# yccyenchicheng/p2pvg

Hardware: NVIDIA H100
Metric: frames/sec (train step, device-timed) MovingMNIST 64x64 seq30 (higher is better)
Workload: dtype bf16

## Files before the change

### p2pvg_b200/csrc/conv_gemm.cu

```cuda
#include <cstdlib>
#include <mutex>

#include "tc_common.cuh"

namespace {

using namespace tc;

constexpr int BLOCK_M = 128;
constexpr int NUM_THREADS = 384;
constexpr int A_STAGE_BYTES = BLOCK_M * 128;

template <int BN> struct Cfg {
  static constexpr int B_STAGE_BYTES = BN * 128;
  static constexpr int STAGE_BYTES = A_STAGE_BYTES + B_STAGE_BYTES;
  static constexpr int STAGES = (BN == 128) ? 4 : 7;
  static constexpr int ACC_LD = BN + 4;
  static constexpr int ACC_BYTES = BLOCK_M * ACC_LD * 4;
  static constexpr int SMEM_BYTES = STAGES * STAGE_BYTES + ACC_BYTES + 1024 + 512;
};

struct Geom {
  int N, H, W;
  int Ck, Cn;
  int M;
  int Ntot;
  int bh128, bn128;
  int bh64, bn64;
  int bw64;
  int imgs_per_group;
  int add_bf16;
  int bres;
  int swap;
  int ks, st, sgn;
};

__device__ __forceinline__ void pix_block(int pb, int P, int H, int W, int bh, int bn, int& n0, int& y0) {
  const int HW = H * W;
  if (HW >= P) {
    const int bpi = HW / P;
    n0 = pb / bpi;
    y0 = (pb - n0 * bpi) * bh;
  } else {
    n0 = pb * bn;
    y0 = 0;
  }
}

__device__ __forceinline__ void addend_load64(float4 (&a4)[16], const float* base, long long elem_off, bool is_bf16) {
  if (is_bf16) {
    const uint4* p = reinterpret_cast<const uint4*>(reinterpret_cast<const bf16*>(base) + elem_off);
#pragma unroll
    for (int j = 0; j < 8; j++) {
      const uint4 r = p[j];
      a4[j] = make_float4(__uint_as_float(r.x), __uint_as_float(r.y), __uint_as_float(r.z), __uint_as_float(r.w));
    }
  } else {
    const float4* p = reinterpret_cast<const float4*>(base + elem_off);
#pragma unroll
    for (int j = 0; j < 16; j++) a4[j] = p[j];
  }
}
__device__ __forceinline__ void addend_add32(float (&f)[32], const float4 (&a4)[16], int h, bool is_bf16) {
  if (is_bf16) {
#pragma unroll
    for (int j = 0; j < 4; j++) {
      const float4 r = a4[4 * h + j];
      float v[8];
      unpack16<bf16>(make_uint4(__float_as_uint(r.x), __float_as_uint(r.y), __float_as_uint(r.z), __float_as_uint(r.w)), v);
#pragma unroll
      for (int i = 0; i < 8; i++) f[8 * j + i] += v[i];
    }
  } else {
#pragma unroll
    for (int j = 0; j < 8; j++) {
      const float4 x4 = a4[8 * h + j];
      f[4 * j] += x4.x; f[4 * j + 1] += x4.y; f[4 * j + 2] += x4.z; f[4 * j + 3] += x4.w;
    }
  }
}

template <int KIND, int BN, bool STAT, bool EVAL = false>
__global__ void __launch_bounds__(NUM_THREADS, 1)
conv_gemm_kernel(const __grid_constant__ CUtensorMap tmA, const __grid_constant__ CUtensorMap tmB, void* __restrict__ Cv, int c_bf16,
                 long long ldc, Geom g, int accumulate, const float* __restrict__ bias, const float* __restrict__ addend,
                 const int* __restrict__ grp_src, float* __restrict__ partial, int kb_per_split, int splits,
                 float2* __restrict__ stat_partial, const float* __restrict__ eval_scale, const float* __restrict__ eval_shift, int act) {
  using C_ = Cfg<BN>;
  constexpr bool A_MN = (KIND == 1), B_MN = (KIND != 0);
  extern __shared__ uint8_t smem_raw[];
  uint8_t* smem = reinterpret_cast<uint8_t*>((reinterpret_cast<uintptr_t>(smem_raw) + 1023) & ~(uintptr_t)1023);
  float* accs = reinterpret_cast<float*>(smem + C_::STAGES * C_::STAGE_BYTES);
  uint64_t* full_bar = reinterpret_cast<uint64_t*>(smem + C_::STAGES * C_::STAGE_BYTES + C_::ACC_BYTES);
  uint64_t* empty_bar = full_bar + C_::STAGES;
  uint64_t* acc_full_bar = empty_bar + C_::STAGES;
  uint64_t* acc_empty_bar = acc_full_bar + 1;
  uint64_t* bres_bar = acc_empty_bar + 1;
  const bool bres = (KIND == 0) && (BN == 64) && g.bres != 0;
  constexpr int BRES_B_BYTES = 9 * 64 * 128, BRES_STAGES = 6;
  static_assert(BN != 64 || BRES_B_BYTES + BRES_STAGES * A_STAGE_BYTES <= C_::STAGES * C_::STAGE_BYTES, "resident weights + A ring");

  const int warp = threadIdx.x >> 5, lane = threadIdx.x & 31;
  const int tiles_m = (g.M + BLOCK_M - 1) / BLOCK_M, tiles_n = (g.Ntot + BN - 1) / BN;
  const int tiles_mn = tiles_m * tiles_n;
  const int phases = (KIND == 2) ? 4 : 1;
  const int num_tiles = tiles_mn * splits * phases;
  const int cchunks = g.Ck / 64;
  const int nkb_total = (KIND == 0) ? g.ks * g.ks * cchunks : (KIND == 2) ? 4 * cchunks : (g.N * g.H * g.W + 63) / 64;

  if (threadIdx.x == 0) {
    for (int s = 0; s < C_::STAGES; s++) {
      mbar_init(&full_bar[s], 1);
      mbar_init(&empty_bar[s], 128);
    }
    mbar_init(acc_full_bar, 128);
    mbar_init(acc_empty_bar, 4);
    mbar_init(bres_bar, 1);
    asm volatile("fence.mbarrier_init.release.cluster;" ::: "memory");
  }
  __syncthreads();

  if (warp >= 8) {
    regs_producer();
    if (warp == 8 && lane == 0) {
      uint32_t it = 0;
      if (bres) {
        mbar_expect_tx(bres_bar, (uint32_t)(g.ks * g.ks) * 64 * 128);
        for (int tap = 0; tap < g.ks * g.ks; tap++) tma_load_2d(&tmB, bres_bar, smem + tap * 64 * 128, tap * 64, 0);
      }
      for (int t = blockIdx.x; t < num_tiles; t += gridDim.x) {
        const int ph = (KIND == 2) ? (t & 3) : 0;
        const int t2 = (KIND == 2) ? (t >> 2) : t;
        const int z = (splits == 1) ? 0 : t2 / tiles_mn, r = t2 - z * tiles_mn;
        const int mt = (tiles_n == 1) ? r : r / tiles_n, nt = (tiles_n == 1) ? 0 : r - mt * tiles_n;
        const int n0 = nt * BN;
        const int kb0 = z * kb_per_split, kb1 = min(kb0 + kb_per_split, nkb_total);
        int pn0 = 0, py0 = 0;
        if (KIND != 1) pix_block(mt, 128, g.H, g.W, g.bh128, g.bn128, pn0, py0);
        const int pa = ph >> 1, pb_ = ph & 1;
        int kn0 = 0, ky0 = 0, kx0 = 0;
        int t_kh = 0, t_kw = 0, t_cc = 0;
        int qc0[BN / 64], qdx[BN / 64], qdy[BN / 64];
        int mc0[2] = {0, 0}, mdx[2] = {0, 0}, mdy[2] = {0, 0};
        if (KIND == 1) {
          if (g.bw64 < g.W) {
            const int per_row = g.W / g.bw64;
            const int rowi = kb0 / per_row;
            kx0 = (kb0 - rowi * per_row) * g.bw64;
            kn0 = rowi / g.H;
            ky0 = rowi - kn0 * g.H;
          } else {
            pix_block(kb0, 64, g.H, g.W, g.bh64, g.bn64, kn0, ky0);
          }
#pragma unroll
          for (int q = 0; q < BN / 64; q++) {
            const int nb = n0 + 64 * q;
            const int tap = nb / g.Cn;
            const int kh = tap / g.ks;
            qc0[q] = nb - tap * g.Cn;
            qdx[q] = tap - kh * g.ks - 1;
            qdy[q] = kh - 1;
          }
          if (g.swap) {
#pragma unroll
            for (int q = 0; q < 2; q++) {
              const int mb = mt * BLOCK_M + 64 * q;
              int tap = mb / g.Cn;
              if (tap >= g.ks * g.ks) tap = g.ks * g.ks - 1;
              const int kh = tap / g.ks;
              mc0[q] = mb < g.M ? mb - tap * g.Cn : 0;
              mdx[q] = tap - kh * g.ks - 1;
              mdy[q] = kh - 1;
            }
          }
        }
        for (int kb = kb0; kb < kb1; kb++, it++) {
          const int s = bres ? (int)(it % BRES_STAGES) : (int)(it % C_::STAGES);
          const uint32_t par = (bres ? (it / BRES_STAGES) : (it / C_::STAGES)) & 1;
          mbar_wait(&empty_bar[s], par ^ 1);
          uint8_t* sa = bres ? smem + BRES_B_BYTES + s * A_STAGE_BYTES : smem + s * C_::STAGE_BYTES;
          uint8_t* sb = sa + A_STAGE_BYTES;
          mbar_expect_tx(&full_bar[s], bres ? A_STAGE_BYTES : C_::STAGE_BYTES);
          if (KIND == 0) {
            tma_load_4d(&tmA, &full_bar[s], sa, t_cc * 64, g.sgn * (t_kw - 1), g.st * py0 + g.sgn * (t_kh - 1), pn0);
            if (!bres) tma_load_2d(&tmB, &full_bar[s], sb, kb * 64, n0);
            if (++t_cc == cchunks) { t_cc = 0; if (++t_kw == g.ks) { t_kw = 0; t_kh++; } }
          } else if (KIND == 2) {
            const int tq = t_kh, c0 = t_cc * 64;
            if (++t_cc == cchunks) { t_cc = 0; t_kh++; }
            const int i = tq >> 1, j = tq & 1;
            const int dy = i == 0 ? 0 : (pa ? 1 : -1), ky = i == 0 ? pa + 1 : (pa ? 0 : 3);
            const int dx = j == 0 ? 0 : (pb_ ? 1 : -1), kx = j == 0 ? pb_ + 1 : (pb_ ? 0 : 3);
            tma_load_4d(&tmA, &full_bar[s], sa, c0, dx, py0 + dy, pn0);
#pragma unroll
            for (int q = 0; q < BN / 64; q++)
              tma_load_2d(&tmB, &full_bar[s], sb + q * 64 * 128, (ky * 4 + kx) * g.Cn + n0 + 64 * q, c0);
          } else {
            const int m0 = mt * BLOCK_M;
            if (g.swap) {
              tma_load_4d(&tmA, &full_bar[s], sa, mc0[0], g.st * kx0 + mdx[0], g.st * ky0 + mdy[0], kn0);
              tma_load_4d(&tmA, &full_bar[s], sa + 64 * 128, mc0[1], g.st * kx0 + mdx[1], g.st * ky0 + mdy[1], kn0);
#pragma unroll
              for (int q = 0; q < BN / 64; q++) tma_load_2d(&tmB, &full_bar[s], sb + q * 64 * 128, n0 + 64 * q, kb * 64);
            } else {
              tma_load_2d(&tmA, &full_bar[s], sa, m0, kb * 64);
              tma_load_2d(&tmA, &full_bar[s], sa + 64 * 128, m0 + 64, kb * 64);
#pragma unroll
              for (int q = 0; q < BN / 64; q++)
                tma_load_4d(&tmB, &full_bar[s], sb + q * 64 * 128, qc0[q], g.st * kx0 + qdx[q], g.st * ky0 + qdy[q], kn0);
            }
            if (g.bw64 < g.W) {
              kx0 += g.bw64;
              if (kx0 >= g.W) { kx0 = 0; if (++ky0 >= g.H) { ky0 = 0; kn0++; } }
            } else if (g.H * g.W >= 64) {
              ky0 += g.bh64;
              if (ky0 >= g.H) { ky0 = 0; kn0++; }
            } else {
              kn0 += g.bn64;
            }
          }
        }
      }
    }
  } else if (warp >= 4) {
    regs_worker();
    const int wt = threadIdx.x - 128;
    const uint32_t smem0 = smem_u32(smem);
    const uint64_t da0 = A_MN ? make_desc(smem0, 64 * 128, 1024) : make_desc(smem0, 0, 1024);
    const uint64_t db0 = B_MN ? make_desc(smem0 + A_STAGE_BYTES, 64 * 128, 1024) : make_desc(smem0 + A_STAGE_BYTES, 0, 1024);
    uint32_t it = 0, lt = 0;
    if (bres) mbar_wait(bres_bar, 0);
    const uint64_t da0r = make_desc(smem0 + BRES_B_BYTES, 0, 1024), db0r = make_desc(smem0, 0, 1024);
    float acc[2][BN / 2];
    for (int t = blockIdx.x; t < num_tiles; t += gridDim.x, lt++) {
      int z = 0;
      if (splits > 1) z = t / tiles_mn;
      const int kb0 = z * kb_per_split, kb1 = min(kb0 + kb_per_split, nkb_total);
      int prev = -1;
      for (int kb = kb0; kb < kb1; kb++, it++) {
        const int s = bres ? (int)(it % BRES_STAGES) : (int)(it % C_::STAGES);
        const uint32_t par = (bres ? (it / BRES_STAGES) : (it / C_::STAGES)) & 1;
        mbar_wait(&full_bar[s], par);
        const uint64_t stage_off = (uint64_t)((uint32_t)s * (uint32_t)(C_::STAGE_BYTES >> 4));
        const uint64_t a_off = bres ? (uint64_t)((uint32_t)s * (uint32_t)(A_STAGE_BYTES >> 4)) : stage_off;
        const uint64_t b_off = bres ? (uint64_t)((uint32_t)kb * (uint32_t)((64 * 128) >> 4)) : stage_off;
        fence_regs(acc[0]);
        fence_regs(acc[1]);
        wgmma_fence();
        wgmma_kblock<false, BN, A_MN, B_MN>(acc, (bres ? da0r : da0) + a_off, (bres ? db0r : db0) + b_off, kb == kb0);
        wgmma_commit();
        wgmma_wait<1>();
        fence_regs(acc[0]);
        fence_regs(acc[1]);
        if (prev >= 0) mbar_arrive(&empty_bar[prev]);
        prev = s;
      }
      wgmma_wait<0>();
      fence_regs(acc[0]);
      fence_regs(acc[1]);
      if (prev >= 0) mbar_arrive(&empty_bar[prev]);
      mbar_wait(acc_empty_bar, (lt & 1) ^ 1);
      acc_to_smem<BN>(acc, accs, C_::ACC_LD, wt);
      mbar_arrive(acc_full_bar);
    }
  } else {
    regs_worker();
    const int q = warp;
    __shared__ float bias_s[2 * BN];
    __shared__ float2 stat_s[STAT ? 2 * 4 * BN : 1];
    constexpr bool do_stat = STAT;
    __shared__ float ev_s[EVAL ? 2 * 2 * BN : 1];
    uint32_t lt = 0;
    for (int t = blockIdx.x; t < num_tiles; t += gridDim.x, lt++) {
      const int ph = (KIND == 2) ? (t & 3) : 0;
      const int t2 = (KIND == 2) ? (t >> 2) : t;
      const int z = (splits == 1) ? 0 : t2 / tiles_mn, r = t2 - z * tiles_mn;
      const int mt = (tiles_n == 1) ? r : r / tiles_n, nt = (tiles_n == 1) ? 0 : r - mt * tiles_n;
      const int n0 = nt * BN;
      const uint32_t acc = lt & 1;
      const int rt = q * 32 + lane;
      long long out_row = (long long)mt * BLOCK_M + rt;
      long long add_row = 0;
      bool row_ok = out_row < g.M;
      if (KIND == 2) {
        int pn0, py0;
        pix_block(mt, 128, g.H, g.W, g.bh128, g.bn128, pn0, py0);
        const int HW = g.H * g.W;
        int nn, yy, xx;
        if (HW >= 128) { nn = 0; yy = rt / g.W; xx = rt - yy * g.W; }
        else { nn = rt / HW; const int rem = rt - nn * HW; yy = rem / g.W; xx = rem - yy * g.W; }
        const int n = pn0 + nn, y = py0 + yy;
        row_ok = (n < g.N) && (y < g.H);
        const int oy = 2 * y + (ph >> 1), ox = 2 * xx + (ph & 1);
        out_row = ((long long)n * (2 * g.H) + oy) * (2 * g.W) + ox;
        if (addend && row_ok) {
          const int n2 = grp_src[n / g.imgs_per_group] * g.imgs_per_group + (n % g.imgs_per_group);
          add_row = ((long long)n2 * (2 * g.H) + oy) * (2 * g.W) + ox;
        }
      }
      if (KIND == 0 && addend && row_ok) {
        const int HW = g.H * g.W;
        const int n = (int)(out_row / HW);
        const int n2 = grp_src[n / g.imgs_per_group] * g.imgs_per_group + (n % g.imgs_per_group);
        add_row = (long long)n2 * HW + (out_row - (long long)n * HW);
      }
      if (EVAL) {
        for (int i = q * 32 + lane; i < BN; i += 128) {
          const bool in = n0 + i < g.Ntot;
          ev_s[acc * 2 * BN + i] = in ? eval_scale[n0 + i] : 0.f;
          ev_s[acc * 2 * BN + BN + i] = in ? eval_shift[n0 + i] : 0.f;
        }
        if (bias == nullptr) epi_bar_sync();
      }
      if (bias != nullptr) {
        for (int i = q * 32 + lane; i < BN; i += 128) bias_s[acc * BN + i] = (n0 + i < g.Ntot) ? bias[n0 + i] : 0.f;
        epi_bar_sync();
      }
      const bool use_add = (KIND != 1) && addend != nullptr && row_ok;
      const long long aoff0 = add_row * g.Ntot + n0;
      const bool abf = g.add_bf16 != 0;
      float4 a4[16];
      if (use_add) addend_load64(a4, addend, aoff0, abf);
      mbar_wait(acc_full_bar, lt & 1);
#pragma unroll 1
      for (int pr = 0; pr < BN / 64; pr++) {
        if (pr > 0 && use_add) addend_load64(a4, addend, aoff0 + pr * 64, abf);
#pragma unroll
        for (int h = 0; h < 2; h++) {
          const int c = pr * 2 + h;
          uint32_t v[32];
          acc_row32(accs + rt * C_::ACC_LD + c * 32, v);
          if (c == BN / 32 - 1) {
            __syncwarp();
            if (lane == 0) mbar_arrive(acc_empty_bar);
          }
          const int nbase = n0 + c * 32;
          if (nbase >= g.Ntot) continue;
          if (!row_ok && !do_stat) continue;
          if (KIND == 1 && partial != nullptr) {
            float* dst = partial + ((long long)z * g.M + out_row) * g.Ntot + nbase;
#pragma unroll
            for (int j = 0; j < 32; j += 8)
              st_global_256(dst + j, v[j], v[j + 1], v[j + 2], v[j + 3], v[j + 4], v[j + 5], v[j + 6], v[j + 7]);
            continue;
          }
          float f[32];
#pragma unroll
          for (int j = 0; j < 32; j++) f[j] = __uint_as_float(v[j]);
          if (bias) {
            const float* bs = bias_s + acc * BN + c * 32;
#pragma unroll
            for (int j = 0; j < 32; j += 4) {
              const float4 b4 = *reinterpret_cast<const float4*>(bs + j);
              f[j] += b4.x; f[j + 1] += b4.y; f[j + 2] += b4.z; f[j + 3] += b4.w;
            }
          }
          if (use_add) addend_add32(f, a4, h, abf);
          if (EVAL) {
            const float* sc = ev_s + acc * 2 * BN + c * 32;
#pragma unroll
            for (int j = 0; j < 32; j++) {
              float y = fmaf(f[j], sc[j], sc[BN + j]);
              if (act == P2PVG_ACT_LRELU) y = y > 0.f ? y : 0.2f * y;
              else if (act == P2PVG_ACT_TANH) y = tanhf(y);
              f[j] = y;
            }
          }
          if (STAT) {
            float s1[32], s2[32];
#pragma unroll
            for (int j = 0; j < 32; j++) {
              const float r = row_ok ? (c_bf16 ? bf16_round(f[j]) : f[j]) : 0.f;
              s1[j] = r;
              s2[j] = r * r;
            }
            const float cs = warp_colsum32(s1, lane), cq = warp_colsum32(s2, lane);
            stat_s[(acc * 4 + q) * BN + c * 32 + lane] = make_float2(cs, cq);
            if (!row_ok) continue;
          }
          if (c_bf16) {
            bf16* crow = reinterpret_cast<bf16*>(Cv) + out_row * ldc + nbase;
            if (accumulate) {
#pragma unroll
              for (int j = 0; j < 32; j++) f[j] += __bfloat162float(crow[j]);
            }
            if ((reinterpret_cast<uintptr_t>(crow) & 31) == 0) {
#pragma unroll
              for (int j = 0; j < 32; j += 16)
                st_global_256(crow + j, pack_bf16x2(f[j], f[j + 1]), pack_bf16x2(f[j + 2], f[j + 3]), pack_bf16x2(f[j + 4], f[j + 5]),
                              pack_bf16x2(f[j + 6], f[j + 7]), pack_bf16x2(f[j + 8], f[j + 9]), pack_bf16x2(f[j + 10], f[j + 11]),
                              pack_bf16x2(f[j + 12], f[j + 13]), pack_bf16x2(f[j + 14], f[j + 15]));
            } else {
#pragma unroll
              for (int j = 0; j < 32; j += 8) {
                uint4 pk;
                pk.x = pack_bf16x2(f[j], f[j + 1]);
                pk.y = pack_bf16x2(f[j + 2], f[j + 3]);
                pk.z = pack_bf16x2(f[j + 4], f[j + 5]);
                pk.w = pack_bf16x2(f[j + 6], f[j + 7]);
                *reinterpret_cast<uint4*>(crow + j) = pk;
              }
            }
          } else {
            float* crow = reinterpret_cast<float*>(Cv) + out_row * ldc + nbase;
            if (accumulate) {
#pragma unroll
              for (int j = 0; j < 32; j++) f[j] += crow[j];
            }
            if ((reinterpret_cast<uintptr_t>(crow) & 31) == 0) {
#pragma unroll
              for (int j = 0; j < 32; j += 8)
                st_global_256(crow + j, __float_as_uint(f[j]), __float_as_uint(f[j + 1]), __float_as_uint(f[j + 2]), __float_as_uint(f[j + 3]),
                              __float_as_uint(f[j + 4]), __float_as_uint(f[j + 5]), __float_as_uint(f[j + 6]), __float_as_uint(f[j + 7]));
            } else {
#pragma unroll
              for (int j = 0; j < 32; j += 4) *reinterpret_cast<float4*>(crow + j) = make_float4(f[j], f[j + 1], f[j + 2], f[j + 3]);
            }
          }
        }
      }
      if (STAT) {
        epi_bar_sync();
        float2* dst = stat_partial + ((long long)mt * phases + ph) * g.Ntot + n0;
        for (int i = q * 32 + lane; i < BN; i += 128) {
          if (n0 + i >= g.Ntot) continue;
          const float2 a = stat_s[(acc * 4 + 0) * BN + i], b = stat_s[(acc * 4 + 1) * BN + i];
          const float2 c2 = stat_s[(acc * 4 + 2) * BN + i], d = stat_s[(acc * 4 + 3) * BN + i];
          dst[i] = make_float2((a.x + b.x) + (c2.x + d.x), (a.y + b.y) + (c2.y + d.y));
        }
      }
    }
  }
}

__global__ void conv_splitk_reduce_kernel(const float* __restrict__ partial, int splits, float* __restrict__ C, long long ldc, int M, int N,
                                          int accumulate, int transposed) {
  const long long total = (long long)M * N;
  for (long long idx = (long long)blockIdx.x * blockDim.x + threadIdx.x; idx < total; idx += (long long)gridDim.x * blockDim.x) {
    const long long m = idx / N;
    const int n = (int)(idx - m * N);
    const long long pidx = transposed ? (long long)n * M + m : idx;
    float acc = 0.f;
    for (int z = 0; z < splits; z++) acc += partial[(long long)z * total + pidx];
    if (accumulate) acc += C[m * ldc + n];
    C[m * ldc + n] = acc;
  }
}

typedef CUresult (*EncodeTiledFn)(CUtensorMap*, CUtensorMapDataType, cuuint32_t, void*, const cuuint64_t*, const cuuint64_t*,
                                  const cuuint32_t*, const cuuint32_t*, CUtensorMapInterleave, CUtensorMapSwizzle,
                                  CUtensorMapL2promotion, CUtensorMapFloatOOBfill);
EncodeTiledFn g_enc = nullptr;
std::once_flag g_once2;
int g_sms = 132;
int g_attr[3][3][2] = {};
int g_bres = 1;
int g_k1_swap = 1;

void resolve2() {
  int dev = 0, sms = 0;
  if (cudaGetDevice(&dev) == cudaSuccess && cudaDeviceGetAttribute(&sms, cudaDevAttrMultiProcessorCount, dev) == cudaSuccess && sms > 0) g_sms = sms;
  void* fn = nullptr;
  cudaDriverEntryPointQueryResult q;
  if (cudaGetDriverEntryPoint("cuTensorMapEncodeTiled", &fn, cudaEnableDefault, &q) == cudaSuccess && q == cudaDriverEntryPointSuccess)
    g_enc = reinterpret_cast<EncodeTiledFn>(fn);
  (void)cudaGetLastError();
  const char* br = getenv("P2PVG_CONV_BRES");
  if (br != nullptr && br[0] == '0') g_bres = 0;
  const char* sw = getenv("P2PVG_K1_SWAP");
  if (sw != nullptr && sw[0] == '0') g_k1_swap = 0;
}

int map2d(CUtensorMap* m, const void* base, long long dim0, long long dim1, long long ld, int box1) {
  cuuint64_t dims[2] = {(cuuint64_t)dim0, (cuuint64_t)dim1};
  cuuint64_t strides[1] = {(cuuint64_t)ld * 2};
  cuuint32_t box[2] = {64, (cuuint32_t)box1};
  cuuint32_t es[2] = {1, 1};
  CUresult r = g_enc(m, CU_TENSOR_MAP_DATA_TYPE_BFLOAT16, 2, const_cast<void*>(base), dims, strides, box, es, CU_TENSOR_MAP_INTERLEAVE_NONE,
                     CU_TENSOR_MAP_SWIZZLE_128B, CU_TENSOR_MAP_L2_PROMOTION_L2_256B, CU_TENSOR_MAP_FLOAT_OOB_FILL_NONE);
  if (r != CUDA_SUCCESS) {
    p2pvg_set_error("conv_gemm: 2-D tensor map failed (%d)", (int)r);
    return P2PVG_ERR_CUDA;
  }
  return P2PVG_OK;
}

int map4d(CUtensorMap* m, const void* base, int N, int Hm, int Wm, int C, int bw, int bh, int bn, int s) {
  cuuint64_t dims[4] = {(cuuint64_t)C, (cuuint64_t)Wm, (cuuint64_t)Hm, (cuuint64_t)N};
  cuuint64_t strides[3] = {(cuuint64_t)C * 2, (cuuint64_t)Wm * C * 2, (cuuint64_t)Hm * Wm * C * 2};
  cuuint32_t box[4] = {64, (cuuint32_t)(bw * s), (cuuint32_t)(bh * s), (cuuint32_t)bn};
  cuuint32_t es[4] = {1, (cuuint32_t)s, (cuuint32_t)s, 1};
  CUresult r = g_enc(m, CU_TENSOR_MAP_DATA_TYPE_BFLOAT16, 4, const_cast<void*>(base), dims, strides, box, es, CU_TENSOR_MAP_INTERLEAVE_NONE,
                     CU_TENSOR_MAP_SWIZZLE_128B, CU_TENSOR_MAP_L2_PROMOTION_L2_256B, CU_TENSOR_MAP_FLOAT_OOB_FILL_NONE);
  if (r != CUDA_SUCCESS) {
    p2pvg_set_error("conv_gemm: 4-D tensor map failed (%d): N=%d H=%d W=%d C=%d box=(%d,%d,%d) s=%d", (int)r, N, Hm, Wm, C, bw, bh, bn, s);
    return P2PVG_ERR_CUDA;
  }
  return P2PVG_OK;
}

bool box_for(int P, int H, int W, int& bh, int& bn) {
  const int HW = H * W;
  if (HW >= P) {
    if (P % W != 0 || (H % (P / W)) != 0) return false;
    bh = P / W;
    bn = 1;
  } else {
    if (P % HW != 0) return false;
    bh = H;
    bn = P / HW;
  }
  return bh * 2 <= 256 && W * 2 <= 256 && bn <= 256;
}

struct EvalEpi {
  const float* scale = nullptr;
  const float* shift = nullptr;
  int act = 0;
};

template <int KIND, int BN, bool STAT, bool EVAL>
int launch_t(const CUtensorMap& ta, const CUtensorMap& tb, void* C, int c_dtype, long long ldc, const Geom& g, int accumulate,
             const float* bias, const float* addend, const int* grp_src, float* partial, int splits, int kb_per_split, cudaStream_t st,
             float2* stat_partial, const EvalEpi& ev);

template <int KIND, int BN>
int launch(const CUtensorMap& ta, const CUtensorMap& tb, void* C, int c_dtype, long long ldc, const Geom& g, int accumulate,
           const float* bias, const float* addend, const int* grp_src, float* partial, int splits, int kb_per_split, cudaStream_t st,
           float2* stat_partial = nullptr, const EvalEpi& ev = EvalEpi()) {
  if (KIND != 1 && ev.scale != nullptr) return launch_t<KIND, BN, false, (KIND != 1)>(ta, tb, C, c_dtype, ldc, g, accumulate, bias, addend, grp_src, partial, splits, kb_per_split, st, nullptr, ev);
  if (KIND != 1 && stat_partial != nullptr) return launch_t<KIND, BN, (KIND != 1), false>(ta, tb, C, c_dtype, ldc, g, accumulate, bias, addend, grp_src, partial, splits, kb_per_split, st, stat_partial, ev);
  return launch_t<KIND, BN, false, false>(ta, tb, C, c_dtype, ldc, g, accumulate, bias, addend, grp_src, partial, splits, kb_per_split, st, nullptr, ev);
}

template <int KIND, int BN, bool STAT, bool EVAL>
int launch_t(const CUtensorMap& ta, const CUtensorMap& tb, void* C, int c_dtype, long long ldc, const Geom& g, int accumulate,
             const float* bias, const float* addend, const int* grp_src, float* partial, int splits, int kb_per_split, cudaStream_t st,
             float2* stat_partial, const EvalEpi& ev) {
  auto kern = conv_gemm_kernel<KIND, BN, STAT, EVAL>;
  int& done = g_attr[EVAL ? 2 : STAT][KIND][BN == 128];
  if (!done) {
    cudaError_t e = cudaFuncSetAttribute(kern, cudaFuncAttributeMaxDynamicSharedMemorySize, Cfg<BN>::SMEM_BYTES);
    if (e != cudaSuccess) {
      p2pvg_set_error("conv_gemm: cudaFuncSetAttribute: %s", cudaGetErrorString(e));
      return P2PVG_ERR_CUDA;
    }
    done = 1;
  }
  long long tiles = (long long)cdiv(g.M, BLOCK_M) * cdiv(g.Ntot, BN) * splits * (KIND == 2 ? 4 : 1);
  int grid = (int)(tiles < g_sms ? tiles : g_sms);
  kern<<<grid, NUM_THREADS, Cfg<BN>::SMEM_BYTES, st>>>(ta, tb, C, c_dtype == P2PVG_BF16, ldc, g, accumulate, bias, addend, grp_src, partial,
                                                      kb_per_split, splits, stat_partial, ev.scale, ev.shift, ev.act);
  return p2pvg_check_launch("conv_gemm");
}

}

int p2pvg_conv_gemm_impl(int kind, const void* a, const void* b, long long ldb, void* c, int c_dtype, long long ldc, int N, int H, int W,
                         int Ck, int Cn, int Cm, const float* bias, const float* addend, const int* grp_src, int imgs_per_group,
                         int accumulate, void* ws, size_t ws_bytes, void* stat_partial_v, int addend_dtype, const float* eval_scale,
                         const float* eval_shift, int act, cudaStream_t st) {
  float2* stat_partial = reinterpret_cast<float2*>(stat_partial_v);
  EvalEpi ev;
  ev.scale = eval_scale; ev.shift = eval_shift; ev.act = act;
  std::call_once(g_once2, resolve2);
  P2PVG_REQUIRE(g_enc != nullptr, P2PVG_ERR_UNSUPPORTED, "conv_gemm: cuTensorMapEncodeTiled unavailable");
  P2PVG_REQUIRE(kind >= 0 && kind <= 5, P2PVG_ERR_BAD_ARG, "conv_gemm: bad kind %d", kind);
  if (eval_scale != nullptr) {
    P2PVG_REQUIRE(kind == 0 || kind == 2, P2PVG_ERR_BAD_ARG, "conv_gemm: the eval-BatchNorm epilogue belongs to kinds 0 and 2");
    P2PVG_REQUIRE(eval_shift != nullptr, P2PVG_ERR_BAD_ARG, "conv_gemm: eval_scale without eval_shift");
    P2PVG_REQUIRE(stat_partial == nullptr, P2PVG_ERR_BAD_ARG, "conv_gemm: the eval-BatchNorm epilogue excludes fwd_stat_partial");
    P2PVG_REQUIRE(!accumulate, P2PVG_ERR_BAD_ARG, "conv_gemm: the eval-BatchNorm epilogue does not accumulate");
    P2PVG_REQUIRE(act == P2PVG_ACT_LRELU || act == P2PVG_ACT_TANH, P2PVG_ERR_BAD_ARG, "conv_gemm: eval epilogue act %d", act);
  }
  if (N <= 0) return P2PVG_OK;
  Geom g;
  g.N = N; g.H = H; g.W = W; g.Ck = Ck; g.Cn = Cn; g.imgs_per_group = imgs_per_group > 0 ? imgs_per_group : 1;
  g.add_bf16 = (addend != nullptr && addend_dtype == P2PVG_BF16) ? 1 : 0;
  g.swap = 0;
  g.bres = 0;
  g.ks = kind >= 3 ? 3 : 4; g.st = kind >= 3 ? 1 : 2; g.sgn = kind == 5 ? -1 : 1;
  const int taps = g.ks * g.ks;
  if (kind == 3 || kind == 5) kind = 0;
  if (kind == 4) kind = 1;
  g.bh128 = g.bn128 = g.bh64 = g.bn64 = 1;
  g.bw64 = W;
  bool ok;
  if (kind == 1) {
    if (W > 64 && W % 64 == 0 && W * g.st <= 256) { g.bw64 = 64; ok = true; }
    else ok = box_for(64, H, W, g.bh64, g.bn64);
  } else {
    ok = box_for(128, H, W, g.bh128, g.bn128);
  }
  ok = ok && (((uintptr_t)a | (uintptr_t)b | (uintptr_t)c) & 15) == 0;
  if (kind == 1) ok = ok && (Cn % 64 == 0) && (Cm % 8 == 0);
  else ok = ok && (Ck % 64 == 0) && (Cn % 32 == 0) && (ldb % 8 == 0);
  if (kind == 2 || addend != nullptr) ok = ok && (Cn % 64 == 0);
  if (!ok) {
    p2pvg_set_error("conv_gemm: shape not supported by the pixel-box tiling (kind=%d N=%d H=%d W=%d Ck=%d Cn=%d)", kind, N, H, W, Ck, Cn);
    return P2PVG_ERR_UNSUPPORTED;
  }
  CUtensorMap ta, tb;
  int rc;
  const long long pix = (long long)N * H * W;
  if (kind == 0) {
    g.M = (int)pix; g.Ntot = Cn;
    rc = map4d(&ta, a, N, g.st * H, g.st * W, Ck, W, g.bh128, g.bn128, g.st);
    if (rc) return rc;
    const int BN = Cn > 64 ? 128 : 64;
    rc = map2d(&tb, b, (long long)taps * Ck, Cn, ldb, BN);
    if (rc) return rc;
    const int nkb = taps * (Ck / 64);
    g.bres = (BN == 64 && Cn == 64 && Ck == 64 && taps <= 9 && g_bres) ? 1 : 0;
    if (BN == 128) return launch<0, 128>(ta, tb, c, c_dtype, ldc, g, accumulate, bias, addend, grp_src, nullptr, 1, nkb, st, stat_partial, ev);
    return launch<0, 64>(ta, tb, c, c_dtype, ldc, g, accumulate, bias, addend, grp_src, nullptr, 1, nkb, st, stat_partial, ev);
  }
  if (kind == 2) {
    g.M = (int)pix; g.Ntot = Cn;
    rc = map4d(&ta, a, N, H, W, Ck, W, g.bh128, g.bn128, 1);
    if (rc) return rc;
    rc = map2d(&tb, b, 16LL * Cn, Ck, ldb, 64);
    if (rc) return rc;
    const int nkb = 4 * (Ck / 64);
    const int BN = Cn > 64 ? 128 : 64;
    if (BN == 128) return launch<2, 128>(ta, tb, c, c_dtype, ldc, g, accumulate, bias, addend, grp_src, nullptr, 1, nkb, st, stat_partial, ev);
    return launch<2, 64>(ta, tb, c, c_dtype, ldc, g, accumulate, bias, addend, grp_src, nullptr, 1, nkb, st, stat_partial, ev);
  }
  P2PVG_REQUIRE(c_dtype == P2PVG_F32, P2PVG_ERR_BAD_ARG, "conv_gemm kind 1 writes fp32");
  P2PVG_REQUIRE(stat_partial == nullptr, P2PVG_ERR_BAD_ARG, "conv_gemm: BatchNorm statistics belong to the forward / data-gradient kinds");
  g.Ck = 64;
  const int nkb = (int)((pix + 63) / 64);
  g.swap = (Cm == 64 && g_k1_swap && nkb >= 16 && ws != nullptr && (size_t)2 * taps * Cn * Cm * sizeof(float) <= ws_bytes) ? 1 : 0;
  if (g.swap) {
    g.M = taps * Cn; g.Ntot = Cm;
    rc = map4d(&ta, b, N, g.st * H, g.st * W, Cn, g.bw64, g.bh64, g.bn64, g.st);
    if (rc) return rc;
    rc = map2d(&tb, a, Cm, pix, Cm, 64);
    if (rc) return rc;
  } else {
    g.M = Cm; g.Ntot = taps * Cn;
    rc = map2d(&ta, a, Cm, pix, Cm, 64);
    if (rc) return rc;
    rc = map4d(&tb, b, N, g.st * H, g.st * W, Cn, g.bw64, g.bh64, g.bn64, g.st);
    if (rc) return rc;
  }
  const int BN = (g.Ntot % 128 == 0) ? 128 : 64;
  const long long tiles = (long long)cdiv(g.M, BLOCK_M) * cdiv(g.Ntot, BN);
  int splits = g.swap ? 2 : 1;
  {
    double best = 1e300;
    const int maxs = nkb / 8 < 64 ? nkb / 8 : 64;
    const int smin = g.swap ? 2 : 1;
    for (int s = smin; s <= (maxs < smin ? smin : maxs); s++) {
      const int kb = cdiv(nkb, s), se = cdiv(nkb, kb);
      if (se > 1 && (ws == nullptr || (size_t)se * g.M * g.Ntot * sizeof(float) > ws_bytes)) continue;
      const long long rounds = cdiv((long long)tiles * se, g_sms);
      double cost = (double)rounds * (kb + 8.0);
      if (se > 1) cost += (double)se * g.M * g.Ntot * 8.0 / 6.0e12 / (0.22e-6 * BN / 128);
      if (cost < best) { best = cost; splits = se; }
    }
  }
  int kbps = cdiv(nkb, splits);
  splits = cdiv(nkb, kbps);
  float* partial = splits > 1 ? reinterpret_cast<float*>(ws) : nullptr;
  if (BN == 128) rc = launch<1, 128>(ta, tb, c, c_dtype, ldc, g, accumulate, nullptr, nullptr, nullptr, partial, splits, kbps, st);
  else rc = launch<1, 64>(ta, tb, c, c_dtype, ldc, g, accumulate, nullptr, nullptr, nullptr, partial, splits, kbps, st);
  if (rc) return rc;
  if (splits > 1) {
    long long total = (long long)Cm * taps * Cn;
    int blocks = (int)((total + 255) / 256 > g_sms * 8 ? g_sms * 8 : (total + 255) / 256);
    conv_splitk_reduce_kernel<<<blocks, 256, 0, st>>>(partial, splits, (float*)c, ldc, Cm, taps * Cn, accumulate, g.swap);
    return p2pvg_check_launch("conv_splitk_reduce");
  }
  P2PVG_REQUIRE(!g.swap, P2PVG_ERR_UNSUPPORTED, "conv_gemm kind 1 (swapped roles) needs the split-K workspace");
  return P2PVG_OK;
}
```

Baseline: 169,700.

## Keep transposed-conv phase weights resident and reuse A halo rows across taps

For the phase-decomposed transposed convolution (kind 2, BN=64), each CTA now handles a fixed output phase. It loads that phase's weight slices into shared memory once and streams only A tiles that are one row taller. Two taps share each A load by shifting the descriptor one row, which halves A traffic and removes repeated B loads. Tiles are also reordered group-minor when an addend is present. The cost is a larger shared memory footprint, a grid rounded down to a multiple of four, and more complex ring and parity bookkeeping that could deadlock or misalign if the geometry assumptions fail.

Result: faster. 174,500 (median of 6 runs) (+2.8%).

```diff
diff --git a/p2pvg_b200/csrc/conv_gemm.cu b/p2pvg_b200/csrc/conv_gemm.cu
--- a/p2pvg_b200/csrc/conv_gemm.cu
+++ b/p2pvg_b200/csrc/conv_gemm.cu
@@ -19,6 +19,10 @@
   static constexpr int ACC_BYTES = BLOCK_M * ACC_LD * 4;
   static constexpr int SMEM_BYTES = STAGES * STAGE_BYTES + ACC_BYTES + 1024 + 512;
 };
+
+constexpr int RPHASE_RING_BYTES = 184 * 1024;
+constexpr int RPHASE_SMEM_BYTES = RPHASE_RING_BYTES + Cfg<64>::ACC_BYTES + 1024 + 512;
+static_assert(RPHASE_SMEM_BYTES + 22 * 64 * 4 <= 227 * 1024, "resident phase weights + A ring + staging buffer");
 
 struct Geom {
   int N, H, W;
@@ -29,8 +33,10 @@
   int bh64, bn64;
   int bw64;
   int imgs_per_group;
+  int groups, grp_tiles;
   int add_bf16;
   int bres;
+  int rphase;
   int swap;
   int ks, st, sgn;
 };
@@ -45,6 +51,12 @@
     n0 = pb * bn;
     y0 = 0;
   }
+}
+
+__device__ __forceinline__ int group_minor_tile(int s, const Geom& g) {
+  if (g.groups <= 1) return s;
+  const int q = s / g.groups;
+  return (s - q * g.groups) * g.grp_tiles + q;
 }
 
 __device__ __forceinline__ void addend_load64(float4 (&a4)[16], const float* base, long long elem_off, bool is_bf16) {
@@ -90,8 +102,10 @@
   constexpr bool A_MN = (KIND == 1), B_MN = (KIND != 0);
   extern __shared__ uint8_t smem_raw[];
   uint8_t* smem = reinterpret_cast<uint8_t*>((reinterpret_cast<uintptr_t>(smem_raw) + 1023) & ~(uintptr_t)1023);
-  float* accs = reinterpret_cast<float*>(smem + C_::STAGES * C_::STAGE_BYTES);
-  uint64_t* full_bar = reinterpret_cast<uint64_t*>(smem + C_::STAGES * C_::STAGE_BYTES + C_::ACC_BYTES);
+  const bool rphase = (KIND == 2) && (BN == 64) && g.rphase != 0;
+  const int ring_bytes = rphase ? RPHASE_RING_BYTES : C_::STAGES * C_::STAGE_BYTES;
+  float* accs = reinterpret_cast<float*>(smem + ring_bytes);
+  uint64_t* full_bar = reinterpret_cast<uint64_t*>(smem + ring_bytes + C_::ACC_BYTES);
   uint64_t* empty_bar = full_bar + C_::STAGES;
   uint64_t* acc_full_bar = empty_bar + C_::STAGES;
   uint64_t* acc_empty_bar = acc_full_bar + 1;
@@ -128,95 +142,122 @@
         mbar_expect_tx(bres_bar, (uint32_t)(g.ks * g.ks) * 64 * 128);
         for (int tap = 0; tap < g.ks * g.ks; tap++) tma_load_2d(&tmB, bres_bar, smem + tap * 64 * 128, tap * 64, 0);
       }
-      for (int t = blockIdx.x; t < num_tiles; t += gridDim.x) {
-        const int ph = (KIND == 2) ? (t & 3) : 0;
-        const int t2 = (KIND == 2) ? (t >> 2) : t;
-        const int z = (splits == 1) ? 0 : t2 / tiles_mn, r = t2 - z * tiles_mn;
-        const int mt = (tiles_n == 1) ? r : r / tiles_n, nt = (tiles_n == 1) ? 0 : r - mt * tiles_n;
-        const int n0 = nt * BN;
-        const int kb0 = z * kb_per_split, kb1 = min(kb0 + kb_per_split, nkb_total);
-        int pn0 = 0, py0 = 0;
-        if (KIND != 1) pix_block(mt, 128, g.H, g.W, g.bh128, g.bn128, pn0, py0);
-        const int pa = ph >> 1, pb_ = ph & 1;
-        int kn0 = 0, ky0 = 0, kx0 = 0;
-        int t_kh = 0, t_kw = 0, t_cc = 0;
-        int qc0[BN / 64], qdx[BN / 64], qdy[BN / 64];
-        int mc0[2] = {0, 0}, mdx[2] = {0, 0}, mdy[2] = {0, 0};
-        if (KIND == 1) {
-          if (g.bw64 < g.W) {
-            const int per_row = g.W / g.bw64;
-            const int rowi = kb0 / per_row;
-            kx0 = (kb0 - rowi * per_row) * g.bw64;
-            kn0 = rowi / g.H;
-            ky0 = rowi - kn0 * g.H;
-          } else {
-            pix_block(kb0, 64, g.H, g.W, g.bh64, g.bn64, kn0, ky0);
-          }
-#pragma unroll
-          for (int q = 0; q < BN / 64; q++) {
-            const int nb = n0 + 64 * q;
-            const int tap = nb / g.Cn;
-            const int kh = tap / g.ks;
-            qc0[q] = nb - tap * g.Cn;
-            qdx[q] = tap - kh * g.ks - 1;
-            qdy[q] = kh - 1;
-          }
-          if (g.swap) {
-#pragma unroll
-            for (int q = 0; q < 2; q++) {
-              const int mb = mt * BLOCK_M + 64 * q;
-              int tap = mb / g.Cn;
-              if (tap >= g.ks * g.ks) tap = g.ks * g.ks - 1;
+      if (rphase) {
+        const int ph = blockIdx.x & 3, pa = ph >> 1, pb_ = ph & 1;
+        mbar_expect_tx(bres_bar, (uint32_t)(4 * cchunks) * 64 * 128);
+        for (int tq = 0, kb = 0; tq < 4; tq++) {
+          const int i = tq >> 1, j = tq & 1;
+          const int ky = i == 0 ? pa + 1 : (pa ? 0 : 3), kx = j == 0 ? pb_ + 1 : (pb_ ? 0 : 3);
+          for (int c = 0; c < cchunks; c++, kb++) tma_load_2d(&tmB, bres_bar, smem + kb * 64 * 128, (ky * 4 + kx) * g.Cn, c * 64);
+        }
+        uint8_t* ring = smem + cchunks * 4 * 64 * 128;
+        const uint32_t abytes = (uint32_t)(g.bh128 + 1) * g.W * 128;
+        int s = 0;
+        uint32_t par = 0;
+        for (int t = blockIdx.x; t < num_tiles; t += gridDim.x) {
+          int pn0, py0;
+          pix_block(group_minor_tile(t >> 2, g), 128, g.H, g.W, g.bh128, g.bn128, pn0, py0);
+          for (int j = 0; j < 2; j++) {
+            const int dx = j == 0 ? 0 : (pb_ ? 1 : -1);
+            for (int c = 0; c < cchunks; c++) {
+              mbar_wait(&empty_bar[s], par ^ 1);
+              mbar_expect_tx(&full_bar[s], abytes);
+              tma_load_4d(&tmA, &full_bar[s], ring + s * abytes, c * 64, dx, py0 - 1 + pa, pn0);
+              if (++s == g.rphase) { s = 0; par ^= 1; }
+            }
+          }
+        }
+      } else {
+        for (int t = blockIdx.x; t < num_tiles; t += gridDim.x) {
+          const int ph = (KIND == 2) ? (t & 3) : 0;
+          const int t2 = (KIND == 2) ? (t >> 2) : t;
+          const int z = (splits == 1) ? 0 : t2 / tiles_mn, r = t2 - z * tiles_mn;
+          const int mt = (tiles_n == 1) ? r : r / tiles_n, nt = (tiles_n == 1) ? 0 : r - mt * tiles_n;
+          const int n0 = nt * BN;
+          const int kb0 = z * kb_per_split, kb1 = min(kb0 + kb_per_split, nkb_total);
+          int pn0 = 0, py0 = 0;
+          if (KIND != 1) pix_block(KIND == 2 ? group_minor_tile(mt, g) : mt, 128, g.H, g.W, g.bh128, g.bn128, pn0, py0);
+          const int pa = ph >> 1, pb_ = ph & 1;
+          int kn0 = 0, ky0 = 0, kx0 = 0;
+          int t_kh = 0, t_kw = 0, t_cc = 0;
+          int qc0[BN / 64], qdx[BN / 64], qdy[BN / 64];
+          int mc0[2] = {0, 0}, mdx[2] = {0, 0}, mdy[2] = {0, 0};
+          if (KIND == 1) {
+            if (g.bw64 < g.W) {
+              const int per_row = g.W / g.bw64;
+              const int rowi = kb0 / per_row;
+              kx0 = (kb0 - rowi * per_row) * g.bw64;
+              kn0 = rowi / g.H;
+              ky0 = rowi - kn0 * g.H;
+            } else {
+              pix_block(kb0, 64, g.H, g.W, g.bh64, g.bn64, kn0, ky0);
+            }
+#pragma unroll
+            for (int q = 0; q < BN / 64; q++) {
+              const int nb = n0 + 64 * q;
+              const int tap = nb / g.Cn;
               const int kh = tap / g.ks;
-              mc0[q] = mb < g.M ? mb - tap * g.Cn : 0;
-              mdx[q] = tap - kh * g.ks - 1;
-              mdy[q] = kh - 1;
-            }
-          }
-        }
-        for (int kb = kb0; kb < kb1; kb++, it++) {
-          const int s = bres ? (int)(it % BRES_STAGES) : (int)(it % C_::STAGES);
-          const uint32_t par = (bres ? (it / BRES_STAGES) : (it / C_::STAGES)) & 1;
-          mbar_wait(&empty_bar[s], par ^ 1);
-          uint8_t* sa = bres ? smem + BRES_B_BYTES + s * A_STAGE_BYTES : smem + s * C_::STAGE_BYTES;
-          uint8_t* sb = sa + A_STAGE_BYTES;
-          mbar_expect_tx(&full_bar[s], bres ? A_STAGE_BYTES : C_::STAGE_BYTES);
-          if (KIND == 0) {
-            tma_load_4d(&tmA, &full_bar[s], sa, t_cc * 64, g.sgn * (t_kw - 1), g.st * py0 + g.sgn * (t_kh - 1), pn0);
-            if (!bres) tma_load_2d(&tmB, &full_bar[s], sb, kb * 64, n0);
-            if (++t_cc == cchunks) { t_cc = 0; if (++t_kw == g.ks) { t_kw = 0; t_kh++; } }
-          } else if (KIND == 2) {
-            const int tq = t_kh, c0 = t_cc * 64;
-            if (++t_cc == cchunks) { t_cc = 0; t_kh++; }
-            const int i = tq >> 1, j = tq & 1;
-            const int dy = i == 0 ? 0 : (pa ? 1 : -1), ky = i == 0 ? pa + 1 : (pa ? 0 : 3);
-            const int dx = j == 0 ? 0 : (pb_ ? 1 : -1), kx = j == 0 ? pb_ + 1 : (pb_ ? 0 : 3);
-            tma_load_4d(&tmA, &full_bar[s], sa, c0, dx, py0 + dy, pn0);
-#pragma unroll
-            for (int q = 0; q < BN / 64; q++)
-              tma_load_2d(&tmB, &full_bar[s], sb + q * 64 * 128, (ky * 4 + kx) * g.Cn + n0 + 64 * q, c0);
-          } else {
-            const int m0 = mt * BLOCK_M;
+              qc0[q] = nb - tap * g.Cn;
+              qdx[q] = tap - kh * g.ks - 1;
+              qdy[q] = kh - 1;
+            }
             if (g.swap) {
-              tma_load_4d(&tmA, &full_bar[s], sa, mc0[0], g.st * kx0 + mdx[0], g.st * ky0 + mdy[0], kn0);
-              tma_load_4d(&tmA, &full_bar[s], sa + 64 * 128, mc0[1], g.st * kx0 + mdx[1], g.st * ky0 + mdy[1], kn0);
-#pragma unroll
-              for (int q = 0; q < BN / 64; q++) tma_load_2d(&tmB, &full_bar[s], sb + q * 64 * 128, n0 + 64 * q, kb * 64);
+#pragma unroll
+              for (int q = 0; q < 2; q++) {
+                const int mb = mt * BLOCK_M + 64 * q;
+                int tap = mb / g.Cn;
+                if (tap >= g.ks * g.ks) tap = g.ks * g.ks - 1;
+                const int kh = tap / g.ks;
+                mc0[q] = mb < g.M ? mb - tap * g.Cn : 0;
+                mdx[q] = tap - kh * g.ks - 1;
+                mdy[q] = kh - 1;
+              }
+            }
+          }
+          for (int kb = kb0; kb < kb1; kb++, it++) {
+            const int s = bres ? (int)(it % BRES_STAGES) : (int)(it % C_::STAGES);
+            const uint32_t par = (bres ? (it / BRES_STAGES) : (it / C_::STAGES)) & 1;
+            mbar_wait(&empty_bar[s], par ^ 1);
+            uint8_t* sa = bres ? smem + BRES_B_BYTES + s * A_STAGE_BYTES : smem + s * C_::STAGE_BYTES;
+            uint8_t* sb = sa + A_STAGE_BYTES;
+            mbar_expect_tx(&full_bar[s], bres ? A_STAGE_BYTES : C_::STAGE_BYTES);
+            if (KIND == 0) {
+              tma_load_4d(&tmA, &full_bar[s], sa, t_cc * 64, g.sgn * (t_kw - 1), g.st * py0 + g.sgn * (t_kh - 1), pn0);
+              if (!bres) tma_load_2d(&tmB, &full_bar[s], sb, kb * 64, n0);
+              if (++t_cc == cchunks) { t_cc = 0; if (++t_kw == g.ks) { t_kw = 0; t_kh++; } }
+            } else if (KIND == 2) {
+              const int tq = t_kh, c0 = t_cc * 64;
+              if (++t_cc == cchunks) { t_cc = 0; t_kh++; }
+              const int i = tq >> 1, j = tq & 1;
+              const int dy = i == 0 ? 0 : (pa ? 1 : -1), ky = i == 0 ? pa + 1 : (pa ? 0 : 3);
+              const int dx = j == 0 ? 0 : (pb_ ? 1 : -1), kx = j == 0 ? pb_ + 1 : (pb_ ? 0 : 3);
+              tma_load_4d(&tmA, &full_bar[s], sa, c0, dx, py0 + dy, pn0);
+#pragma unroll
+              for (int q = 0; q < BN / 64; q++)
+                tma_load_2d(&tmB, &full_bar[s], sb + q * 64 * 128, (ky * 4 + kx) * g.Cn + n0 + 64 * q, c0);
             } else {
-              tma_load_2d(&tmA, &full_bar[s], sa, m0, kb * 64);
-              tma_load_2d(&tmA, &full_bar[s], sa + 64 * 128, m0 + 64, kb * 64);
-#pragma unroll
-              for (int q = 0; q < BN / 64; q++)
-                tma_load_4d(&tmB, &full_bar[s], sb + q * 64 * 128, qc0[q], g.st * kx0 + qdx[q], g.st * ky0 + qdy[q], kn0);
-            }
-            if (g.bw64 < g.W) {
-              kx0 += g.bw64;
-              if (kx0 >= g.W) { kx0 = 0; if (++ky0 >= g.H) { ky0 = 0; kn0++; } }
-            } else if (g.H * g.W >= 64) {
-              ky0 += g.bh64;
-              if (ky0 >= g.H) { ky0 = 0; kn0++; }
-            } else {
-              kn0 += g.bn64;
+              const int m0 = mt * BLOCK_M;
+              if (g.swap) {
+                tma_load_4d(&tmA, &full_bar[s], sa, mc0[0], g.st * kx0 + mdx[0], g.st * ky0 + mdy[0], kn0);
+                tma_load_4d(&tmA, &full_bar[s], sa + 64 * 128, mc0[1], g.st * kx0 + mdx[1], g.st * ky0 + mdy[1], kn0);
+#pragma unroll
+                for (int q = 0; q < BN / 64; q++) tma_load_2d(&tmB, &full_bar[s], sb + q * 64 * 128, n0 + 64 * q, kb * 64);
+              } else {
+                tma_load_2d(&tmA, &full_bar[s], sa, m0, kb * 64);
+                tma_load_2d(&tmA, &full_bar[s], sa + 64 * 128, m0 + 64, kb * 64);
+#pragma unroll
+                for (int q = 0; q < BN / 64; q++)
+                  tma_load_4d(&tmB, &full_bar[s], sb + q * 64 * 128, qc0[q], g.st * kx0 + qdx[q], g.st * ky0 + qdy[q], kn0);
+              }
+              if (g.bw64 < g.W) {
+                kx0 += g.bw64;
+                if (kx0 >= g.W) { kx0 = 0; if (++ky0 >= g.H) { ky0 = 0; kn0++; } }
+              } else if (g.H * g.W >= 64) {
+                ky0 += g.bh64;
+                if (ky0 >= g.H) { ky0 = 0; kn0++; }
+              } else {
+                kn0 += g.bn64;
+              }
             }
           }
         }
@@ -229,8 +270,13 @@
     const uint64_t da0 = A_MN ? make_desc(smem0, 64 * 128, 1024) : make_desc(smem0, 0, 1024);
     const uint64_t db0 = B_MN ? make_desc(smem0 + A_STAGE_BYTES, 64 * 128, 1024) : make_desc(smem0 + A_STAGE_BYTES, 0, 1024);
     uint32_t it = 0, lt = 0;
-    if (bres) mbar_wait(bres_bar, 0);
+    if (bres || rphase) mbar_wait(bres_bar, 0);
     const uint64_t da0r = make_desc(smem0 + BRES_B_BYTES, 0, 1024), db0r = make_desc(smem0, 0, 1024);
+    const int half = 2 * cchunks, pa = (blockIdx.x & 3) >> 1;
+    const uint64_t da0p = make_desc(smem0 + 4 * cchunks * 64 * 128, 0, 1024), db0p = make_desc(smem0, 64 * 128, 1024);
+    const uint32_t box16 = (uint32_t)(g.bh128 + 1) * g.W * 8, row16 = (uint32_t)g.W * 8;
+    int s0 = 0;
+    uint32_t par0 = 0;
     float acc[2][BN / 2];
     for (int t = blockIdx.x; t < num_tiles; t += gridDim.x, lt++) {
       int z = 0;
@@ -238,27 +284,43 @@
       const int kb0 = z * kb_per_split, kb1 = min(kb0 + kb_per_split, nkb_total);
       int prev = -1;
       for (int kb = kb0; kb < kb1; kb++, it++) {
-        const int s = bres ? (int)(it % BRES_STAGES) : (int)(it % C_::STAGES);
-        const uint32_t par = (bres ? (it / BRES_STAGES) : (it / C_::STAGES)) & 1;
-        mbar_wait(&full_bar[s], par);
+        int s;
+        uint32_t par;
+        bool reuse = false;
+        if (rphase) {
+          reuse = kb >= half;
+          s = s0 + kb - (reuse ? half : 0);
+          par = par0;
+          if (s >= g.rphase) { s -= g.rphase; par ^= 1; }
+        } else {
+          s = bres ? (int)(it % BRES_STAGES) : (int)(it % C_::STAGES);
+          par = (bres ? (it / BRES_STAGES) : (it / C_::STAGES)) & 1;
+        }
+        if (!reuse) mbar_wait(&full_bar[s], par);
         const uint64_t stage_off = (uint64_t)((uint32_t)s * (uint32_t)(C_::STAGE_BYTES >> 4));
         const uint64_t a_off = bres ? (uint64_t)((uint32_t)s * (uint32_t)(A_STAGE_BYTES >> 4)) : stage_off;
         const uint64_t b_off = bres ? (uint64_t)((uint32_t)kb * (uint32_t)((64 * 128) >> 4)) : stage_off;
+        uint64_t da = (bres ? da0r : da0) + a_off, db = (bres ? db0r : db0) + b_off;
+        if (rphase) {
+          da = da0p + (uint64_t)((uint32_t)s * box16 + (reuse == (pa != 0) ? row16 : 0u));
+          db = db0p + (uint64_t)((uint32_t)kb * (uint32_t)((64 * 128) >> 4));
+        }
         fence_regs(acc[0]);
         fence_regs(acc[1]);
         wgmma_fence();
-        wgmma_kblock<false, BN, A_MN, B_MN>(acc, (bres ? da0r : da0) + a_off, (bres ? db0r : db0) + b_off, kb == kb0);
+        wgmma_kblock<false, BN, A_MN, B_MN>(acc, da, db, kb == kb0);
         wgmma_commit();
         wgmma_wait<1>();
         fence_regs(acc[0]);
         fence_regs(acc[1]);
         if (prev >= 0) mbar_arrive(&empty_bar[prev]);
-        prev = s;
+        prev = (rphase && !reuse) ? -1 : s;
       }
       wgmma_wait<0>();
       fence_regs(acc[0]);
       fence_regs(acc[1]);
       if (prev >= 0) mbar_arrive(&empty_bar[prev]);
+      if (rphase && (s0 += half) >= g.rphase) { s0 -= g.rphase; par0 ^= 1; }
       mbar_wait(acc_empty_bar, (lt & 1) ^ 1);
       acc_to_smem<BN>(acc, accs, C_::ACC_LD, wt);
       mbar_arrive(acc_full_bar);
@@ -275,7 +337,8 @@
       const int ph = (KIND == 2) ? (t & 3) : 0;
       const int t2 = (KIND == 2) ? (t >> 2) : t;
       const int z = (splits == 1) ? 0 : t2 / tiles_mn, r = t2 - z * tiles_mn;
-      const int mt = (tiles_n == 1) ? r : r / tiles_n, nt = (tiles_n == 1) ? 0 : r - mt * tiles_n;
+      const int ms = (tiles_n == 1) ? r : r / tiles_n, nt = (tiles_n == 1) ? 0 : r - ms * tiles_n;
+      const int mt = (KIND == 2) ? group_minor_tile(ms, g) : ms;
       const int n0 = nt * BN;
       const uint32_t acc = lt & 1;
       const int rt = q * 32 + lane;
@@ -538,19 +601,24 @@
              const float* bias, const float* addend, const int* grp_src, float* partial, int splits, int kb_per_split, cudaStream_t st,
              float2* stat_partial, const EvalEpi& ev) {
   auto kern = conv_gemm_kernel<KIND, BN, STAT, EVAL>;
+  constexpr bool can_rphase = (KIND == 2) && (BN == 64);
+  constexpr int max_smem = (can_rphase && RPHASE_SMEM_BYTES > Cfg<BN>::SMEM_BYTES) ? RPHASE_SMEM_BYTES : Cfg<BN>::SMEM_BYTES;
   int& done = g_attr[EVAL ? 2 : STAT][KIND][BN == 128];
   if (!done) {
-    cudaError_t e = cudaFuncSetAttribute(kern, cudaFuncAttributeMaxDynamicSharedMemorySize, Cfg<BN>::SMEM_BYTES);
+    cudaError_t e = cudaFuncSetAttribute(kern, cudaFuncAttributeMaxDynamicSharedMemorySize, max_smem);
     if (e != cudaSuccess) {
       p2pvg_set_error("conv_gemm: cudaFuncSetAttribute: %s", cudaGetErrorString(e));
       return P2PVG_ERR_CUDA;
     }
     done = 1;
   }
+  const bool rphase = can_rphase && g.rphase != 0;
   long long tiles = (long long)cdiv(g.M, BLOCK_M) * cdiv(g.Ntot, BN) * splits * (KIND == 2 ? 4 : 1);
   int grid = (int)(tiles < g_sms ? tiles : g_sms);
-  kern<<<grid, NUM_THREADS, Cfg<BN>::SMEM_BYTES, st>>>(ta, tb, C, c_dtype == P2PVG_BF16, ldc, g, accumulate, bias, addend, grp_src, partial,
-                                                      kb_per_split, splits, stat_partial, ev.scale, ev.shift, ev.act);
+  if (rphase) grid &= ~3;
+  const int smem = rphase ? RPHASE_SMEM_BYTES : Cfg<BN>::SMEM_BYTES;
+  kern<<<grid, NUM_THREADS, smem, st>>>(ta, tb, C, c_dtype == P2PVG_BF16, ldc, g, accumulate, bias, addend, grp_src, partial,
+                                        kb_per_split, splits, stat_partial, ev.scale, ev.shift, ev.act);
   return p2pvg_check_launch("conv_gemm");
 }
 
@@ -579,6 +647,8 @@
   g.add_bf16 = (addend != nullptr && addend_dtype == P2PVG_BF16) ? 1 : 0;
   g.swap = 0;
   g.bres = 0;
+  g.rphase = 0;
+  g.groups = g.grp_tiles = 0;
   g.ks = kind >= 3 ? 3 : 4; g.st = kind >= 3 ? 1 : 2; g.sgn = kind == 5 ? -1 : 1;
   const int taps = g.ks * g.ks;
   if (kind == 3 || kind == 5) kind = 0;
@@ -617,12 +687,22 @@
   }
   if (kind == 2) {
     g.M = (int)pix; g.Ntot = Cn;
-    rc = map4d(&ta, a, N, H, W, Ck, W, g.bh128, g.bn128, 1);
+    const int nkb = 4 * (Ck / 64);
+    const int BN = Cn > 64 ? 128 : 64;
+    if (BN == 64 && g.bn128 == 1 && W % 8 == 0) {
+      const int wbytes = nkb * 64 * 128, abytes = (g.bh128 + 1) * W * 128;
+      const int stages = wbytes < RPHASE_RING_BYTES ? (RPHASE_RING_BYTES - wbytes) / abytes : 0;
+      if (stages > nkb / 2) g.rphase = stages < Cfg<64>::STAGES ? stages : Cfg<64>::STAGES;
+    }
+    const long long grp_pix = (long long)g.imgs_per_group * H * W;
+    if (addend != nullptr && N % g.imgs_per_group == 0 && grp_pix % BLOCK_M == 0) {
+      g.groups = N / g.imgs_per_group;
+      g.grp_tiles = (int)(grp_pix / BLOCK_M);
+    }
+    rc = map4d(&ta, a, N, H, W, Ck, W, g.bh128 + (g.rphase ? 1 : 0), g.bn128, 1);
     if (rc) return rc;
     rc = map2d(&tb, b, 16LL * Cn, Ck, ldb, 64);
     if (rc) return rc;
-    const int nkb = 4 * (Ck / 64);
-    const int BN = Cn > 64 ? 128 : 64;
     if (BN == 128) return launch<2, 128>(ta, tb, c, c_dtype, ldc, g, accumulate, bias, addend, grp_src, nullptr, 1, nkb, st, stat_partial, ev);
     return launch<2, 64>(ta, tb, c, c_dtype, ldc, g, accumulate, bias, addend, grp_src, nullptr, 1, nkb, st, stat_partial, ev);
   }
```
